# FluidInference/FluidAudio

Measured on NVIDIA H100. Metric: audio-hours/s, higher is better.
Workload: dtype f32

## Files before the change

fluidaudio_b200/csrc/mel_core.cuh:

```cuda
#pragma once

#include "fa_common.cuh"
#include <math.h>
#include <stdint.h>

namespace fa {
namespace mel {

constexpr int kNfft = 512;
constexpr int kHalf = 256;
constexpr int kBins = 257;
constexpr int kFftPad = 304;
constexpr int kTileFrames = 16;
constexpr int kWarpsPerCta = 8;
constexpr int kPairStride = 524;
FA_HD int pow_pos(int bin) { return bin ^ ((bin >> 4) & 3); }

struct alignas(8) cpx {
    float x, y;
};

struct alignas(8) f32x2 {
    float a, b;
};

#if defined(__CUDA_ARCH__)
__device__ __forceinline__ float2 as_f2(f32x2 v) { return make_float2(v.a, v.b); }
__device__ __forceinline__ f32x2 as_v(float2 v) {
    f32x2 r;
    r.a = v.x;
    r.b = v.y;
    return r;
}
#endif

FA_HD double vadd(double x, double y) { return x + y; }
FA_HD double vsub(double x, double y) { return x - y; }
FA_HD double vneg(double x) { return -x; }
FA_HD double vmul_s(double x, double s) { return x * s; }
FA_HD double vfma_s(double a, double s, double c) { return a * s + c; }
FA_HD double vfnma_s(double a, double s, double c) { return c - a * s; }

FA_HD f32x2 vneg(f32x2 x) {
    f32x2 r;
    r.a = -x.a;
    r.b = -x.b;
    return r;
}
#if defined(__CUDA_ARCH__)
__device__ __forceinline__ f32x2 vadd(f32x2 x, f32x2 y) { return as_v(fadd2_rn(as_f2(x), as_f2(y))); }
__device__ __forceinline__ f32x2 vsub(f32x2 x, f32x2 y) { return as_v(fadd2_rn(as_f2(x), as_f2(vneg(y)))); }
__device__ __forceinline__ f32x2 vmul_s(f32x2 x, float s) { return as_v(fmul2_rn(as_f2(x), make_float2(s, s))); }
__device__ __forceinline__ f32x2 vfma_s(f32x2 a, float s, f32x2 c) {
    return as_v(ffma2_rn(as_f2(a), make_float2(s, s), as_f2(c)));
}
__device__ __forceinline__ f32x2 vfnma_s(f32x2 a, float s, f32x2 c) {
    return as_v(ffma2_rn(as_f2(vneg(a)), make_float2(s, s), as_f2(c)));
}
#else
inline f32x2 vadd(f32x2 x, f32x2 y) { return f32x2{x.a + y.a, x.b + y.b}; }
inline f32x2 vsub(f32x2 x, f32x2 y) { return f32x2{x.a - y.a, x.b - y.b}; }
inline f32x2 vmul_s(f32x2 x, float s) { return f32x2{x.a * s, x.b * s}; }
inline f32x2 vfma_s(f32x2 a, float s, f32x2 c) { return f32x2{fmaf(a.a, s, c.a), fmaf(a.b, s, c.b)}; }
inline f32x2 vfnma_s(f32x2 a, float s, f32x2 c) { return f32x2{fmaf(-a.a, s, c.a), fmaf(-a.b, s, c.b)}; }
#endif

template <typename V>
struct vtraits;
template <>
struct vtraits<double> {
    typedef double scalar;
    static constexpr int kFrames = 1;
};
template <>
struct vtraits<f32x2> {
    typedef float scalar;
    static constexpr int kFrames = 2;
};

template <typename V>
struct alignas(16) cpxv {
    V x, y;
};
typedef cpxv<double> cpxd;
struct cpxs {
    float x, y;
};

struct LaneCommon {
    float win[16];
    uint32_t in_win;
    int a1, a2, k0;
    int k0s, kc0s;
};
template <typename V>
struct LaneTables;
template <>
struct LaneTables<double> : LaneCommon {
    cpxd w256;
    cpxd w32;
    cpxd wk0;
};
template <>
struct LaneTables<f32x2> : LaneCommon {
    cpxs tw1[8];
    cpxs tw2[8];
    cpxs wk[4];
};

FA_HD void lane_butterflies(int l, int &c1, int &c2) {
    if (l >= 8) {
        c1 = l;
        c2 = 8 * (8 - (l >> 3)) + (7 - (l & 7));
    } else if (l >= 4) {
        c1 = 32 + (l - 4);
        c2 = 39 - (l - 4);
    } else if (l >= 1) {
        c1 = l;
        c2 = 8 - l;
    } else {
        c1 = 0;
        c2 = 4;
    }
}

FA_HD cpxd unit_root(int k, int n) {
    const double a = -6.283185307179586476925286766559 * (double)k / (double)n;
    cpxd r;
    r.x = cos(a);
    r.y = sin(a);
    return r;
}
FA_HD cpxs unit_root_f(int k, int n) {
    const cpxd d = unit_root(k, n);
    cpxs r;
    r.x = (float)d.x;
    r.y = (float)d.y;
    return r;
}

FA_HD void load_lane_common(int l, const float *win_tab, const uint8_t *in_tab, LaneCommon &T) {
    T.in_win = 0;
#pragma unroll
    for (int r = 0; r < 8; ++r) {
        const int j = 2 * (l + 32 * r);
        T.win[2 * r] = win_tab[j];
        T.win[2 * r + 1] = win_tab[j + 1];
        if (in_tab[j]) T.in_win |= 1u << (2 * r);
        if (in_tab[j + 1]) T.in_win |= 1u << (2 * r + 1);
    }
    int c1, c2;
    lane_butterflies(l, c1, c2);
    T.a1 = 9 * (c1 >> 3) + (c1 & 7);
    T.a2 = 9 * (c2 >> 3) + (c2 & 7);
    T.k0 = (c1 >> 3) + 8 * (c1 & 7);
    T.k0s = pow_pos(T.k0);
    T.kc0s = pow_pos(kHalf - T.k0);
}
FA_HD void load_lane_tables(int l, const float *win_tab, const uint8_t *in_tab, LaneTables<double> &T) {
    load_lane_common(l, win_tab, in_tab, T);
    T.w256 = unit_root(l, 256);
    T.w32 = unit_root(l & 3, 32);
    T.wk0 = unit_root(T.k0, 512);
}
FA_HD void load_lane_tables(int l, const float *win_tab, const uint8_t *in_tab, LaneTables<f32x2> &T) {
    load_lane_common(l, win_tab, in_tab, T);
#pragma unroll
    for (int q = 0; q < 8; ++q) {
        T.tw1[q] = unit_root_f((l * q) & 255, 256);
        T.tw2[q] = unit_root_f(((l & 3) * q) & 31, 32);
    }
#pragma unroll
    for (int k2 = 0; k2 < 4; ++k2) T.wk[k2] = unit_root_f(T.k0 + 64 * k2, 512);
}

FA_HD cpxd cmul(cpxd a, cpxd b) {
    cpxd r;
    r.x = a.x * b.x - a.y * b.y;
    r.y = a.x * b.y + a.y * b.x;
    return r;
}

template <typename V>
FA_HD void dft4(V &r0, V &i0, V &r1, V &i1, V &r2, V &i2, V &r3, V &i3) {
    const V ar = vadd(r0, r2), ai = vadd(i0, i2);
    const V br = vsub(r0, r2), bi = vsub(i0, i2);
    const V cr = vadd(r1, r3), ci = vadd(i1, i3);
    const V dr = vsub(r1, r3), di = vsub(i1, i3);
    r0 = vadd(ar, cr);
    i0 = vadd(ai, ci);
    r2 = vsub(ar, cr);
    i2 = vsub(ai, ci);
    r1 = vadd(br, di);
    i1 = vsub(bi, dr);
    r3 = vsub(br, di);
    i3 = vadd(bi, dr);
}

template <typename V>
FA_HD void dft8(V (&re)[8], V (&im)[8]) {
    typedef typename vtraits<V>::scalar S;
    const S kS = (S)0.70710678118654752440;
    V er0 = vadd(re[0], re[4]), ei0 = vadd(im[0], im[4]);
    V er1 = vadd(re[1], re[5]), ei1 = vadd(im[1], im[5]);
    V er2 = vadd(re[2], re[6]), ei2 = vadd(im[2], im[6]);
    V er3 = vadd(re[3], re[7]), ei3 = vadd(im[3], im[7]);
    V or0 = vsub(re[0], re[4]), oi0 = vsub(im[0], im[4]);
    const V xr1 = vsub(re[1], re[5]), xi1 = vsub(im[1], im[5]);
    const V xr2 = vsub(re[2], re[6]), xi2 = vsub(im[2], im[6]);
    const V xr3 = vsub(re[3], re[7]), xi3 = vsub(im[3], im[7]);
    V or1 = vmul_s(vadd(xr1, xi1), kS), oi1 = vmul_s(vsub(xi1, xr1), kS);
    V or2 = xi2, oi2 = vneg(xr2);
    V or3 = vmul_s(vsub(xi3, xr3), kS), oi3 = vmul_s(vadd(xr3, xi3), (S)(-kS));
    dft4(er0, ei0, er1, ei1, er2, ei2, er3, ei3);
    dft4(or0, oi0, or1, oi1, or2, oi2, or3, oi3);
    re[0] = er0; im[0] = ei0;
    re[2] = er1; im[2] = ei1;
    re[4] = er2; im[4] = ei2;
    re[6] = er3; im[6] = ei3;
    re[1] = or0; im[1] = oi0;
    re[3] = or1; im[3] = oi1;
    re[5] = or2; im[5] = oi2;
    re[7] = or3; im[7] = oi3;
}

template <typename Emit>
FA_HD void twiddle_emit(double (&re)[8], double (&im)[8], cpxd root, Emit emit) {
    cpxd p[8];
    p[1] = root;
    p[2] = cmul(root, root);
    p[3] = cmul(p[2], root);
    p[4] = cmul(p[2], p[2]);
    p[5] = cmul(p[4], root);
    p[6] = cmul(p[4], p[2]);
    p[7] = cmul(p[4], p[3]);
    cpxd v;
    v.x = re[0];
    v.y = im[0];
    emit(0, v);
#pragma unroll
    for (int q = 1; q < 8; ++q) {
        v.x = re[q] * p[q].x - im[q] * p[q].y;
        v.y = re[q] * p[q].y + im[q] * p[q].x;
        emit(q, v);
    }
}
template <typename Emit>
FA_HD void twiddle_emit(f32x2 (&re)[8], f32x2 (&im)[8], const cpxs (&tw)[8], Emit emit) {
    cpxv<f32x2> v;
    v.x = re[0];
    v.y = im[0];
    emit(0, v);
#pragma unroll
    for (int q = 1; q < 8; ++q) {
        v.x = vfnma_s(im[q], tw[q].y, vmul_s(re[q], tw[q].x));
        v.y = vfma_s(im[q], tw[q].x, vmul_s(re[q], tw[q].y));
        emit(q, v);
    }
}
FA_HD void twiddle_pass1(int l, double (&re)[8], double (&im)[8], const LaneTables<double> &T, cpxd *buf) {
    twiddle_emit(re, im, T.w256, [&](int q, cpxd v) { buf[l + 36 * q] = v; });
}
FA_HD void twiddle_pass1(int l, f32x2 (&re)[8], f32x2 (&im)[8], const LaneTables<f32x2> &T, cpxv<f32x2> *buf) {
    twiddle_emit(re, im, T.tw1, [&](int q, cpxv<f32x2> v) { buf[l + 36 * q] = v; });
}
FA_HD void twiddle_pass2(int base, double (&re)[8], double (&im)[8], const LaneTables<double> &T, cpxd *buf) {
    twiddle_emit(re, im, T.w32, [&](int q2, cpxd v) { buf[base + q2] = v; });
}
FA_HD void twiddle_pass2(int base, f32x2 (&re)[8], f32x2 (&im)[8], const LaneTables<f32x2> &T, cpxv<f32x2> *buf) {
    twiddle_emit(re, im, T.tw2, [&](int q2, cpxv<f32x2> v) { buf[base + q2] = v; });
}

FA_HD void widen(float a, float b, float, float, double &re, double &im) {
    re = (double)a;
    im = (double)b;
}
FA_HD void widen(float a, float b, float a2, float b2, f32x2 &re, f32x2 &im) {
    re.a = a;
    re.b = a2;
    im.a = b;
    im.b = b2;
}

template <bool kMidFull, typename V>
FA_HD void pass1(int l, const float *pf, int hop, const LaneTables<V> &T, cpxv<V> *buf) {
    V re[8], im[8];
#pragma unroll
    for (int r = 0; r < 8; ++r) {
        const int j = 2 * (l + 32 * r);
#if defined(__CUDA_ARCH__)
        const float2 v = *reinterpret_cast<const float2 *>(pf + j);
        float2 u = v;
        if (vtraits<V>::kFrames == 2) u = *reinterpret_cast<const float2 *>(pf + hop + j);
#else
        const cpx v = *reinterpret_cast<const cpx *>(pf + j);
        cpx u = v;
        if (vtraits<V>::kFrames == 2) u = *reinterpret_cast<const cpx *>(pf + hop + j);
#endif
        float a = T.win[2 * r] * v.x, b = T.win[2 * r + 1] * v.y;
        float a2 = T.win[2 * r] * u.x, b2 = T.win[2 * r + 1] * u.y;
        if (!kMidFull || r == 0 || r == 7) {
            const bool ia = (T.in_win >> (2 * r)) & 1u, ib = (T.in_win >> (2 * r + 1)) & 1u;
            a = ia ? a : 0.0f;
            b = ib ? b : 0.0f;
            a2 = ia ? a2 : 0.0f;
            b2 = ib ? b2 : 0.0f;
        }
        widen(a, b, a2, b2, re[r], im[r]);
    }
    dft8(re, im);
    twiddle_pass1(l, re, im, T, buf);
}

template <typename V>
FA_HD void pass2_load(int l, const cpxv<V> *buf, V (&re)[8], V (&im)[8]) {
    const int base = 36 * (l >> 2) + (l & 3);
#pragma unroll
    for (int r = 0; r < 8; ++r) {
        const cpxv<V> v = buf[base + 4 * r];
        re[r] = v.x;
        im[r] = v.y;
    }
}
template <typename V>
FA_HD void pass2_store(int l, const LaneTables<V> &T, V (&re)[8], V (&im)[8], cpxv<V> *buf) {
    dft8(re, im);
    const int base = 74 * (l & 3) + 9 * (l >> 2);
    twiddle_pass2(base, re, im, T, buf);
}

FA_HD void pair_power(double zbx, double zby, double zcx, double zcy, double wx, double wy, float *prow, int ib, int ic) {
    const double sr = zbx + zcx, si = zby - zcy;
    const double dr = zby + zcy, di = zcx - zbx;
    const double tr = wx * dr - wy * di, ti = wx * di + wy * dr;
    const float xr = (float)(sr + tr), xi = (float)(si + ti);
    const float yr = (float)(sr - tr), yi = (float)(si - ti);
#if defined(__CUDA_ARCH__)
    prow[2 * ib] = __fadd_rn(__fmul_rn(xr, xr), __fmul_rn(xi, xi));
    prow[2 * ic] = __fadd_rn(__fmul_rn(yr, yr), __fmul_rn(yi, yi));
#else
    const float a = xr * xr, b = xi * xi, c = yr * yr, d = yi * yi;
    prow[2 * ib] = a + b;
    prow[2 * ic] = c + d;
#endif
}
FA_HD void pair_power(f32x2 zbx, f32x2 zby, f32x2 zcx, f32x2 zcy, float wx, float wy, float *prow, int ib, int ic) {
    const f32x2 sr = vadd(zbx, zcx), si = vsub(zby, zcy);
    const f32x2 dr = vadd(zby, zcy), di = vsub(zcx, zbx);
    const f32x2 tr = vfnma_s(di, wy, vmul_s(dr, wx)), ti = vfma_s(dr, wy, vmul_s(di, wx));
    const f32x2 xr = vadd(sr, tr), xi = vadd(si, ti);
    const f32x2 yr = vsub(sr, tr), yi = vsub(si, ti);
#if defined(__CUDA_ARCH__)
    const float2 pb = ffma2_rn(as_f2(xr), as_f2(xr), fmul2_rn(as_f2(xi), as_f2(xi)));
    const float2 pc = ffma2_rn(as_f2(yr), as_f2(yr), fmul2_rn(as_f2(yi), as_f2(yi)));
    *reinterpret_cast<float2 *>(prow + 2 * ib) = pb;
    *reinterpret_cast<float2 *>(prow + 2 * ic) = pc;
#else
    prow[2 * ib] = fmaf(xr.a, xr.a, xi.a * xi.a);
    prow[2 * ic] = fmaf(yr.a, yr.a, yi.a * yi.a);
    prow[2 * ib + 1] = fmaf(xr.b, xr.b, xi.b * xi.b);
    prow[2 * ic + 1] = fmaf(yr.b, yr.b, yi.b * yi.b);
#endif
}

FA_HD void recombination_roots(const LaneTables<double> &T, double (&wx)[4], double (&wy)[4]) {
    const double hh = 0.70710678118654752440;
    wx[0] = T.wk0.x;
    wy[0] = T.wk0.y;
    wx[1] = hh * (wx[0] + wy[0]);
    wy[1] = hh * (wy[0] - wx[0]);
    wx[2] = wy[0];
    wy[2] = -wx[0];
    wx[3] = wy[1];
    wy[3] = -wx[1];
}
FA_HD void recombination_roots(const LaneTables<f32x2> &T, float (&wx)[4], float (&wy)[4]) {
#pragma unroll
    for (int k = 0; k < 4; ++k) {
        wx[k] = T.wk[k].x;
        wy[k] = T.wk[k].y;
    }
}

template <typename V>
FA_HD void pass3_post(int l, const cpxv<V> *buf, const LaneTables<V> &T, float *prow) {
    typedef typename vtraits<V>::scalar S;
    V ar[4], ai[4], br[4], bi[4];
#pragma unroll
    for (int h = 0; h < 4; ++h) {
        const cpxv<V> u = buf[T.a1 + 74 * h], v = buf[T.a2 + 74 * h];
        ar[h] = u.x;
        ai[h] = u.y;
        br[h] = v.x;
        bi[h] = v.y;
    }
    dft4(ar[0], ai[0], ar[1], ai[1], ar[2], ai[2], ar[3], ai[3]);
    dft4(br[0], bi[0], br[1], bi[1], br[2], bi[2], br[3], bi[3]);
    const bool z = l == 0;
    const S c1 = (S)0.92387953251128675613, s1 = (S)0.38268343236508977173;
    S wx[4], wy[4];
    recombination_roots(T, wx, wy);
    pair_power(ar[0], ai[0], z ? ar[0] : br[3], z ? ai[0] : bi[3], wx[0], wy[0], prow, T.k0s, T.kc0s);
    pair_power(ar[1], ai[1], z ? ar[3] : br[2], z ? ai[3] : bi[2], wx[1], wy[1], prow, T.k0s + 64, T.kc0s - 64);
    pair_power(ar[2], ai[2], z ? ar[2] : br[1], z ? ai[2] : bi[1], wx[2], wy[2], prow, T.k0s + 128, T.kc0s - 128);
    const int b3 = z ? pow_pos(32) : T.k0s + 192, c3 = z ? pow_pos(224) : T.kc0s - 192;
    pair_power(z ? br[0] : ar[3], z ? bi[0] : ai[3], z ? br[3] : br[0], z ? bi[3] : bi[0], z ? c1 : wx[3],
               z ? (S)(-s1) : wy[3], prow, b3, c3);
    if (z) {
        pair_power(br[1], bi[1], br[2], bi[2], s1, (S)(-c1), prow, pow_pos(96), pow_pos(160));
    }
}

FA_HD float mel_dot(const float *prow, const float *w, int lo, int hi) {
    float acc = 0.0f;
    const float *p = prow + lo;
    const int n = hi - lo;
    for (int b = 0; b < n; ++b) {
        const float t = w[b] * p[b];
        acc = acc + t;
    }
    return acc;
}
#if defined(__CUDACC__)
__device__ __forceinline__ float2 mel_dot_pairs(const float4 *p4, const float4 *w4, int nq) {
    float2 acc = make_float2(0.0f, 0.0f);
#pragma unroll 1
    for (int b = 0; b < nq; ++b) {
        const float4 x01 = p4[2 * b], x23 = p4[2 * b + 1], c = w4[b];
        acc = ffma2_rn(make_float2(x01.x, x01.y), make_float2(c.x, c.x), acc);
        acc = ffma2_rn(make_float2(x01.z, x01.w), make_float2(c.y, c.y), acc);
        acc = ffma2_rn(make_float2(x23.x, x23.y), make_float2(c.z, c.z), acc);
        acc = ffma2_rn(make_float2(x23.z, x23.w), make_float2(c.w, c.w), acc);
    }
    return acc;
}
__device__ __forceinline__ float mel_dot_quads(const float4 *p4, const float4 *w4, int nq) {
    float acc = 0.0f;
#pragma unroll 1
    for (int b = 0; b < nq; ++b) {
        const float4 x = p4[b], c = w4[b];
        acc = fmaf(c.x, x.x, acc);
        acc = fmaf(c.y, x.y, acc);
        acc = fmaf(c.z, x.z, acc);
        acc = fmaf(c.w, x.w, acc);
    }
    return acc;
}
#endif

FA_HD float log_value(float v, float floor_, int clamped, int normal_floor = 0) {
    const float x = clamped ? (floor_ >= v ? floor_ : v) : v + floor_;
#if defined(__CUDA_ARCH__)
    float l;
    if (normal_floor) asm("lg2.approx.ftz.f32 %0, %1;" : "=f"(l) : "f"(x));
    else l = __log2f(x);
    return l * 0.693147180559945309417f;
#else
    (void)normal_floor;
    return logf(x);
#endif
}

FA_HD float preemph_first(float x0, float last, float a) {
#if defined(__CUDA_ARCH__)
    return __fsub_rn(x0, __fmul_rn(a, last));
#else
    const float t = a * last;
    return x0 - t;
#endif
}
FA_HD float preemph_rest(float x, float xprev, float a) { return fmaf(xprev, -a, x); }

FA_HD long long reflect_index(long long i, long long n) {
    if (i < 0) return -i < n - 1 ? -i : n - 1;
    if (i >= n) return 2 * n - 2 - i > 0 ? 2 * n - 2 - i : 0;
    return i;
}

}
}
```

fluidaudio_b200/csrc/mel_kernels.cu:

```cuda
#include "mel_core.cuh"
#include "mel_plan.h"

#include <cuda_runtime.h>
#include <algorithm>
#include <cmath>
#include <vector>

namespace fa {
namespace mel {

__device__ __forceinline__ uint32_t smem_u32(const void *p) { return (uint32_t)__cvta_generic_to_shared(p); }

__device__ __forceinline__ void mbar_init(uint64_t *bar, uint32_t count) {
    asm volatile("mbarrier.init.shared::cta.b64 [%0], %1;" ::"r"(smem_u32(bar)), "r"(count));
}
__device__ __forceinline__ void mbar_expect_tx(uint64_t *bar, uint32_t bytes) {
    asm volatile("mbarrier.arrive.expect_tx.shared::cta.b64 _, [%0], %1;" ::"r"(smem_u32(bar)), "r"(bytes) : "memory");
}
__device__ __forceinline__ void mbar_arrive(uint64_t *bar) {
    asm volatile("mbarrier.arrive.shared::cta.b64 _, [%0];" ::"r"(smem_u32(bar)) : "memory");
}
__device__ __forceinline__ bool mbar_try_wait(uint64_t *bar, uint32_t parity) {
    uint32_t ok;
    asm volatile(
        "{\n\t"
        ".reg .pred p;\n\t"
        "mbarrier.try_wait.parity.shared::cta.b64 p, [%1], %2;\n\t"
        "selp.u32 %0, 1, 0, p;\n\t"
        "}"
        : "=r"(ok)
        : "r"(smem_u32(bar)), "r"(parity)
        : "memory");
    return ok != 0;
}
__device__ __forceinline__ void mbar_wait(uint64_t *bar, uint32_t parity) {
    while (!mbar_try_wait(bar, parity)) {
    }
}
__device__ __forceinline__ void bulk_g2s(void *dst, const void *src, uint32_t bytes, uint64_t *bar) {
    asm volatile("cp.async.bulk.shared::cluster.global.mbarrier::complete_tx::bytes [%0], [%1], %2, [%3];" ::"r"(
                     smem_u32(dst)),
                 "l"(src), "r"(bytes), "r"(smem_u32(bar))
                 : "memory");
}
__device__ __forceinline__ void fence_proxy_async() { asm volatile("fence.proxy.async.shared::cta;" ::: "memory"); }

struct TileGeom {
    int unit;
    long long f0;
    int nf;
    long long a0;
    long long base;
    long long gs, ge;
};

__device__ __forceinline__ const MelUnit &unit_at(const MelLaunch &P, int idx) { return P.inline_unit ? P.unit0 : P.units[idx]; }

__device__ __forceinline__ TileGeom tile_geom(const MelLaunch &P, int tile) {
    int lo = 0, hi = P.inline_unit ? 0 : P.num_units - 1;
    while (lo < hi) {
        const int mid = (lo + hi + 1) >> 1;
        if (P.units[mid].tile_begin <= tile) lo = mid; else hi = mid - 1;
    }
    const MelUnit &u = P.inline_unit ? P.unit0 : P.units[lo];
    TileGeom g;
    g.unit = lo;
    g.f0 = u.frame_begin + (long long)kTileFrames * (tile - u.tile_begin);
    const long long rem = u.frame_begin + u.frame_count - g.f0;
    g.nf = rem < kTileFrames ? (int)rem : kTileFrames;
    g.a0 = g.f0 * P.hop - P.pad;
    const long long need0 = g.a0 - 1;
    g.base = (need0 >= 0) ? (need0 & ~3LL) : -(((-need0) + 3) & ~3LL);
    long long ge = (g.a0 + P.pt_len + 3) & ~3LL;
    const long long n4 = u.n & ~3LL;
    if (ge > n4) ge = n4;
    g.gs = g.base < 0 ? 0 : g.base;
    g.ge = ge;
    if (!P.use_tma) g.ge = g.gs;
    return g;
}

struct TileInfo {
    TileGeom g;
    long long audio_off, n, out_off, out_stride;
    float last;
    int pad_;
};
__device__ __forceinline__ void make_tile_info(const MelLaunch &P, int tile, TileInfo &ti) {
    ti.g = tile_geom(P, tile);
    const MelUnit &u = unit_at(P, ti.g.unit);
    ti.audio_off = u.audio_off;
    ti.n = u.n;
    ti.out_off = u.out_off;
    ti.out_stride = u.out_stride;
    ti.last = u.last;
}

template <int kWarps, typename V, int kLayout>
__global__ void __launch_bounds__(kWarps * 32, 2) mel512_kernel(const MelLaunch P) {
    constexpr int kF = vtraits<V>::kFrames;
    extern __shared__ __align__(128) unsigned char smem[];
    float *raw0 = reinterpret_cast<float *>(smem);
    float *raw1 = raw0 + P.raw_cap;
    float *ptile = raw1 + P.raw_cap;
    cpxv<V> *fftbuf = reinterpret_cast<cpxv<V> *>(ptile + P.pt_cap);
    float *power = reinterpret_cast<float *>(fftbuf + kWarps * kFftPad);
    float *otile = power + (kTileFrames / 2) * kPairStride;
    const int ot_stride = P.ot_stride;
    float *fbw = otile + kTileFrames * ot_stride;
    int4 *fbmeta = reinterpret_cast<int4 *>(fbw + P.fb_cap);
    uint64_t *bars = reinterpret_cast<uint64_t *>(fbmeta + P.n_slots);
    TileInfo *tinfo = reinterpret_cast<TileInfo *>(bars + 2);

    const int tid = threadIdx.x, lane = tid & 31, warp = tid >> 5;

    if (tid == 0) {
        mbar_init(&bars[0], 1);
        mbar_init(&bars[1], 1);
        asm volatile("fence.mbarrier_init.release.cluster;" ::: "memory");
    }
    for (int i = tid; i < P.fb_nnz; i += kWarps * 32) fbw[i] = P.fb_w[i];
    for (int i = tid; i < P.n_slots; i += kWarps * 32) fbmeta[i] = P.fb_slots[i];
    for (int i = tid; i < (kTileFrames / 2) * kPairStride; i += kWarps * 32) power[i] = 0.0f;
    const LaneTables<V> T = reinterpret_cast<const LaneTables<V> *>(P.lane_tab)[lane];
    __syncthreads();

    cpxv<V> *buf = fftbuf + warp * kFftPad;

    auto issue = [&](int tile, int buf, TileInfo &slot) {
        make_tile_info(P, tile, slot);
        const TileGeom &g = slot.g;
        float *dst = buf ? raw1 : raw0;
        if (g.ge > g.gs) {
            const uint32_t bytes = (uint32_t)((g.ge - g.gs) * 4);
            mbar_expect_tx(&bars[buf], bytes);
            bulk_g2s(dst + (g.gs - g.base), P.audio + slot.audio_off + g.gs, bytes, &bars[buf]);
        } else {
            mbar_arrive(&bars[buf]);
        }
    };

    auto preemphasize = [&](const TileInfo &u, const float *raw) {
        const TileGeom &g = u.g;
        const float a = P.preemph;
        const bool interior = g.a0 >= 1 && g.a0 - 1 >= g.gs && g.a0 + P.pt_len <= g.ge && g.a0 + P.pt_len <= u.n;
        if (interior) {
            const float *src = raw + (g.a0 - g.base);
            if (((g.a0 - g.base) & 3) == 0 && (P.pt_len & 3) == 0) {
                const float4 *s4 = reinterpret_cast<const float4 *>(src);
                float4 *d4 = reinterpret_cast<float4 *>(ptile);
                for (int q = tid; q < (P.pt_len >> 2); q += kWarps * 32) {
                    const float4 x = s4[q];
                    float4 y = x;
                    const float prev = src[4 * q - 1];
                    if (a != 0.0f) {
                        y.x = preemph_rest(x.x, prev, a);
                        y.y = preemph_rest(x.y, x.x, a);
                        y.z = preemph_rest(x.z, x.y, a);
                        y.w = preemph_rest(x.w, x.z, a);
                    }
                    d4[q] = y;
                }
            } else if (a == 0.0f) {
                for (int t = tid; t < P.pt_len; t += kWarps * 32) ptile[t] = src[t];
            } else {
                for (int t = tid; t < P.pt_len; t += kWarps * 32) ptile[t] = preemph_rest(src[t], src[t - 1], a);
            }
        } else {
            const float *gaudio = P.audio + u.audio_off;
            auto sample = [&](long long i) -> float {
                if (i >= g.gs && i < g.ge) return raw[i - g.base];
                if (i < 0) return u.last;
                return __ldg(gaudio + i);
            };
            for (int t = tid; t < P.pt_len; t += kWarps * 32) {
                const long long i = g.a0 + t;
                float v = 0.0f;
                if (i >= 0 && i < u.n) {
                    const float x = sample(i);
                    if (a == 0.0f) v = x;
                    else if (i == 0) v = preemph_first(x, u.last, a);
                    else v = preemph_rest(x, sample(i - 1), a);
                }
                ptile[t] = v;
            }
        }
    };
    auto copy_out = [&](float *dst, int total) {
        if (P.out_vec4) {
            float4 *d4 = reinterpret_cast<float4 *>(dst);
            for (int q = tid; q < (total >> 2); q += kWarps * 32) {
                const int e = 4 * q;
                const int row = (int)__umulhi((unsigned)e, P.inv_n_mels);
                d4[q] = *reinterpret_cast<const float4 *>(otile + e + 4 * row);
            }
        } else {
            const int row_pad = ot_stride - P.n_mels;
            for (int idx = tid; idx < total; idx += kWarps * 32) {
                const int fi = P.n_mels == 1 ? idx : (int)__umulhi((unsigned)idx, P.inv_n_mels);
                dst[idx] = otile[idx + fi * row_pad];
            }
        }
    };

    const int first = blockIdx.x, stride = gridDim.x;
    if (first >= P.total_tiles) return;
    if (tid == 0) {
        issue(first, 0, tinfo[0]);
        if (first + stride < P.total_tiles) issue(first + stride, 1, tinfo[1]);
    }
    __syncthreads();
    mbar_wait(&bars[0], 0);
    preemphasize(tinfo[0], raw0);
    __syncthreads();
    float *pending_dst = nullptr;
    int pending_total = 0;
    int it = 0, slot = 0;
    for (int tile = first; tile < P.total_tiles; tile += stride, ++it, slot = slot == 2 ? 0 : slot + 1) {
        const TileInfo &u = tinfo[slot];
        const int nf = u.g.nf;

        if (pending_dst) copy_out(pending_dst, pending_total);
        for (int fi = warp * kF; fi < nf; fi += kWarps * kF) {
            const float *pf = ptile + fi * P.hop;
            V re[8], im[8];
            if (P.mid_full) pass1<true>(lane, pf, P.hop, T, buf); else pass1<false>(lane, pf, P.hop, T, buf);
            __syncwarp();
            pass2_load(lane, buf, re, im);
            __syncwarp();
            pass2_store(lane, T, re, im, buf);
            __syncwarp();
            pass3_post(lane, buf, T, power + (fi >> 1) * kPairStride + (fi & 1));
            __syncwarp();
        }
        __syncthreads();

        const int next = tile + stride;
        const int slot1 = slot == 2 ? 0 : slot + 1, slot2 = slot1 == 2 ? 0 : slot1 + 1;
        if (tid == 0 && next + stride < P.total_tiles) {
            fence_proxy_async();
            issue(next + stride, it & 1, tinfo[slot2]);
        }
        {
            constexpr int kPairs = kTileFrames / 2, kGroup = 32 / kPairs;
            const int pl = lane % kPairs, mg = lane / kPairs;
            const float *prow = power + pl * kPairStride;
            float *orow = otile + (2 * pl) * ot_stride;
            float *gout = kLayout == 1 ? P.out + u.out_off + u.g.f0 + 2 * pl : nullptr;
            for (int slot = warp * kGroup + mg; slot < P.n_slots; slot += kWarps * kGroup) {
                const int4 md = fbmeta[slot];
                const float2 a2 = mel_dot_pairs(reinterpret_cast<const float4 *>(prow + 2 * md.x),
                                                reinterpret_cast<const float4 *>(fbw + md.z), md.y);
                const float v0 = log_value(a2.x, P.log_floor, P.log_clamped, P.log_normal),
                            v1 = log_value(a2.y, P.log_floor, P.log_clamped, P.log_normal);
                const int m = md.w;
                if (m < 0) continue;
                if (kLayout == 0) {
                    orow[m] = v0;
                    orow[ot_stride + m] = v1;
                } else {
                    float *g = gout + (long long)m * u.out_stride;
                    if (2 * pl < nf) g[0] = v0;
                    if (2 * pl + 1 < nf) g[1] = v1;
                }
            }
        }
        if (kLayout == 0) {
            pending_dst = P.out + u.out_off + u.g.f0 * P.n_mels;
            pending_total = nf * P.n_mels;
        }
        if (next < P.total_tiles) {
            const int nb = (it + 1) & 1;
            mbar_wait(&bars[nb], (uint32_t)((it + 1) >> 1) & 1u);
            preemphasize(tinfo[slot1], nb ? raw1 : raw0);
        }
        __syncthreads();
    }
    if (pending_dst) copy_out(pending_dst, pending_total);
}


struct GenericParams {
    int n_fft, log2n, bins, prow;
    const cpxd *tw;
    int warps;
    float spectrum_power;
    float log_mean, log_std;
};

template <bool kReflect, int kSpectrum, bool kAffine>
__global__ void __launch_bounds__(256) mel_generic_kernel(const MelLaunch P, const GenericParams G) {
    extern __shared__ __align__(16) unsigned char smem[];
    cpxd *tw = reinterpret_cast<cpxd *>(smem);
    cpxd *fft = tw + G.n_fft / 2;
    float *power = reinterpret_cast<float *>(fft + (size_t)G.warps * G.n_fft);
    float *win = power + (size_t)G.warps * G.prow;
    const int tid = threadIdx.x, lane = tid & 31, warp = tid >> 5, nthreads = G.warps * 32;
    for (int i = tid; i < G.n_fft / 2; i += nthreads) tw[i] = G.tw[i];
    for (int i = tid; i < G.n_fft; i += nthreads) win[i] = P.in_tab[i] ? P.win_tab[i] : 0.0f;
    for (int i = tid; i < G.warps * G.prow; i += nthreads) power[i] = 0.0f;
    __syncthreads();
    cpxd *buf = fft + (size_t)warp * G.n_fft;
    float *prow = power + (size_t)warp * G.prow;
    const float a = P.preemph;
    for (int tile = blockIdx.x; tile < P.total_tiles; tile += gridDim.x) {
        const TileGeom g = tile_geom(P, tile);
        const MelUnit u = unit_at(P, g.unit);
        const float *x = P.audio + u.audio_off;
        for (int fi = warp; fi < g.nf; fi += G.warps) {
            const long long f = g.f0 + fi;
            const long long base = f * P.hop - P.pad;
            for (int j = lane; j < G.n_fft; j += 32) {
                const long long i = base + j;
                float v = 0.0f;
                if (kReflect) {
                    if (u.n > 0 && P.in_tab[j]) v = __fmul_rn(__ldg(x + reflect_index(i, u.n)), win[j]);
                } else if (i >= 0 && i < u.n && P.in_tab[j]) {
                    const float xi = __ldg(x + i);
                    if (a == 0.0f) v = xi;
                    else if (i == 0) v = preemph_first(xi, u.last, a);
                    else v = preemph_rest(xi, __ldg(x + i - 1), a);
                    v = __fmul_rn(v, win[j]);
                }
                cpxd z;
                z.x = (double)v;
                z.y = 0.0;
                buf[__brev((unsigned)j) >> (32 - G.log2n)] = z;
            }
            __syncwarp();
            for (int s = 0; s < G.log2n; ++s) {
                const int half = 1 << s, step = G.n_fft >> (s + 1);
                for (int t = lane; t < G.n_fft / 2; t += 32) {
                    const int j = t & (half - 1);
                    const int ia = ((t >> s) << (s + 1)) + j, ib = ia + half;
                    const cpxd w = tw[j * step], zb = buf[ib], za = buf[ia];
                    const double tr = zb.x * w.x - zb.y * w.y, ti = zb.x * w.y + zb.y * w.x;
                    cpxd o;
                    o.x = za.x - tr;
                    o.y = za.y - ti;
                    buf[ib] = o;
                    o.x = za.x + tr;
                    o.y = za.y + ti;
                    buf[ia] = o;
                }
                __syncwarp();
            }
            for (int b = lane; b < G.bins; b += 32) {
                const float xr = (float)buf[b].x, xi = (float)buf[b].y;
                const float pw = __fadd_rn(__fmul_rn(xr, xr), __fmul_rn(xi, xi));
                if (kSpectrum == kSpecPower) prow[b] = 4.0f * pw;
                else if (kSpectrum == kSpecMagnitude) prow[b] = __fsqrt_rn(pw);
                else prow[b] = powf(__fsqrt_rn(pw), G.spectrum_power);
            }
            __syncwarp();
            for (int m = lane; m < P.n_mels; m += 32) {
                const int lo = P.fb_lo[m], nq = (P.fb_hi[m] - lo) >> 2;
                float v = log_value(mel_dot_quads(reinterpret_cast<const float4 *>(prow + lo),
                                                  reinterpret_cast<const float4 *>(P.fb_w + P.fb_off[m]), nq),
                                    P.log_floor, P.log_clamped);
                if (kAffine) v = __fdiv_rn(__fsub_rn(v, G.log_mean), G.log_std);
                if (P.layout == 0) P.out[u.out_off + f * P.n_mels + m] = v;
                else P.out[u.out_off + (long long)m * u.out_stride + f] = v;
            }
            __syncwarp();
        }
    }
}

static constexpr int kCtasPerSm = 2;

typedef void (*Mel512Kernel)(const MelLaunch);
template <typename V> static Mel512Kernel mel512_variant(int layout) {
    return layout == FA_MEL_TIME_MAJOR ? mel512_kernel<kWarpsPerCta, V, FA_MEL_TIME_MAJOR>
                                       : mel512_kernel<kWarpsPerCta, V, FA_MEL_MEL_MAJOR>;
}
static Mel512Kernel mel512_variant(int precision, int layout) {
    return precision == FA_MEL_PRECISION_F64 ? mel512_variant<double>(layout) : mel512_variant<f32x2>(layout);
}

typedef void (*GenericKernel)(const MelLaunch, const GenericParams);
template <bool R, int S> static GenericKernel generic_variant(bool affine) {
    return affine ? mel_generic_kernel<R, S, true> : mel_generic_kernel<R, S, false>;
}
template <bool R> static GenericKernel generic_variant(int spectrum, bool affine) {
    return spectrum == kSpecPower ? generic_variant<R, kSpecPower>(affine)
                                  : (spectrum == kSpecMagnitude ? generic_variant<R, kSpecMagnitude>(affine)
                                                                : generic_variant<R, kSpecGeneral>(affine));
}
static GenericKernel generic_variant(bool reflect, int spectrum, bool affine) {
    return reflect ? generic_variant<true>(spectrum, affine) : generic_variant<false>(spectrum, affine);
}

static int placement_of(int mode) { return mode == FA_MEL_LEGACY_COMPUTE ? 1 : 0; }
static int window_offset(const MelConfig &c, int placement) { return placement == 1 ? 0 : (c.n_fft - c.win_length) / 2; }

static_assert(sizeof(MelSlot) == sizeof(int4) && offsetof(MelSlot, mel) == offsetof(int4, w), "MelSlot is an int4");

template <typename T, typename U> static int upload_table(DeviceBuffer<T> &b, const std::vector<U> &v) {
    const int st = b.grow(std::max<size_t>(1, v.size()) * sizeof(U));
    if (st != FA_OK) return st;
    if (!v.empty()) FA_CUDA_TRY(cudaMemcpy(b.data(), v.data(), v.size() * sizeof(U), cudaMemcpyHostToDevice));
    return FA_OK;
}

int MelPlan::init(const MelConfig &c) {
    cfg = c;
    if (cfg.pad_to < 1) cfg.pad_to = 1;
    if (cfg.n_mels <= 0 || cfg.hop_length <= 0 || cfg.win_length <= 0 || cfg.n_fft <= 0 || cfg.sample_rate <= 0) {
        fa::set_error("mel config: all sizes must be positive");
        return FA_INVALID_ARGUMENT;
    }
    const bool pow2 = cfg.n_fft >= 32 && cfg.n_fft <= 4096 && (cfg.n_fft & (cfg.n_fft - 1)) == 0;
    if (!pow2 || cfg.win_length > cfg.n_fft || cfg.n_mels > 512 || cfg.hop_length > 65536) {
        fa::set_error("mel config unsupported by the sm_90a kernels: need nFFT a power of two in 32..4096, win <= nFFT, "
                      "nMels <= 512 (got nFFT=%d hop=%d win=%d nMels=%d)",
                      cfg.n_fft, cfg.hop_length, cfg.win_length, cfg.n_mels);
        return FA_UNSUPPORTED;
    }
    if (const char *why = check_ex_config(cfg)) {
        fa::set_error("mel ex config: %s", why);
        return FA_INVALID_ARGUMENT;
    }
    const int spectrum = spectrum_kind(cfg.spectrum_power);
    generic = cfg.n_fft != kNfft || (cfg.hop_length & 1) || cfg.hop_length > 1024 || cfg.reflect() ||
              spectrum != kSpecPower || cfg.affine();
    const int n_fft = cfg.n_fft, bins = n_fft / 2 + 1;
    build_tables(cfg, window, filterbank);
    const MelBands bands = pack_bands(filterbank, cfg.n_mels, bins);
    fb_nnz = bands.nnz;
    n_slots = (int)bands.slots.size();

    int dev = 0;
    FA_CUDA_TRY(cudaGetDevice(&dev));
    cudaDeviceProp prop;
    int st = sm90_device_props(dev, prop);
    if (st != FA_OK) return st;
    num_sms = prop.multiProcessorCount;

    if (!generic) {
        pt_len = (kTileFrames - 1) * cfg.hop_length + kNfft;
        pt_cap = (pt_len + 31) & ~31;
        raw_cap = (pt_len + 1 + 3 + 3 + 31) & ~31;
        fb_cap = (fb_nnz + 3) & ~3;
        smem_bytes = sizeof(float) * ((size_t)2 * raw_cap + pt_cap + 0 +
                                      (size_t)(kTileFrames / 2) * kPairStride + (size_t)kTileFrames * (cfg.n_mels + 4) + fb_cap) +
                     sizeof(cpxd) * (size_t)kWarpsPerCta * kFftPad + sizeof(int) * 4 * (size_t)n_slots + 8 +
                     2 * sizeof(uint64_t) + 3 * sizeof(TileInfo) + 16;
        if (smem_bytes > (size_t)prop.sharedMemPerBlockOptin) {
            generic = true;
            pt_len = pt_cap = raw_cap = fb_cap = 0;
        }
    }

    std::vector<float> win_tab;
    std::vector<uint8_t> in_tab;
    for (int pl = 0; pl < 2; ++pl) {
        place_window(window, n_fft, window_offset(cfg, pl), win_tab, in_tab);
        st = upload_table(d_win_tab_mode[pl], win_tab);
        if (st == FA_OK) st = upload_table(d_in_tab_mode[pl], in_tab);
        if (st != FA_OK) return st;
        if (!generic) {
            std::vector<LaneTables<double>> t64(32);
            std::vector<LaneTables<f32x2>> t32(32);
            for (int l = 0; l < 32; ++l) {
                load_lane_tables(l, win_tab.data(), in_tab.data(), t64[l]);
                load_lane_tables(l, win_tab.data(), in_tab.data(), t32[l]);
            }
            st = upload_table(d_lane_tab[pl][FA_MEL_PRECISION_F64], t64);
            if (st == FA_OK) st = upload_table(d_lane_tab[pl][FA_MEL_PRECISION_F32], t32);
            if (st != FA_OK) return st;
        }
    }
    st = upload_table(d_fb_w, pack_weights(filterbank, bands, bins, !generic, spectrum == kSpecPower ? 0.25f : 1.0f));
    if (st == FA_OK) st = upload_table(d_fb_slots, bands.slots);
    if (st == FA_OK) st = upload_table(d_fb_lo, bands.lo);
    if (st == FA_OK) st = upload_table(d_fb_hi, bands.hi);
    if (st == FA_OK) st = upload_table(d_fb_off, bands.off);
    for (auto &s : streams)
        if (st == FA_OK) st = s.create();
    if (st != FA_OK) return st;
    if (generic) {
        std::vector<cpxd> tw(n_fft / 2);
        for (int k = 0; k < n_fft / 2; ++k) tw[k] = unit_root(k, n_fft);
        st = upload_table(d_generic_tw, tw);
        if (st != FA_OK) return st;
        generic_prow = ((bins + 3) & ~3) + 4;
        int log2n = 0;
        while ((1 << log2n) < n_fft) ++log2n;
        generic_log2n = log2n;
        const size_t fixed = (size_t)(n_fft / 2) * sizeof(cpxd) + (size_t)n_fft * sizeof(float);
        const size_t per_warp = (size_t)n_fft * sizeof(cpxd) + (size_t)generic_prow * sizeof(float);
        generic_warps = (int)std::min<size_t>(8, ((size_t)prop.sharedMemPerBlockOptin - fixed - 1024) / per_warp);
        if (generic_warps < 1) {
            fa::set_error("mel config: nFFT %d does not fit shared memory", n_fft);
            return FA_UNSUPPORTED;
        }
        smem_bytes = fixed + per_warp * generic_warps;
        for (const bool r : {false, cfg.reflect()})
            FA_CUDA_TRY(cudaFuncSetAttribute(generic_variant(r, spectrum, cfg.affine()),
                                             cudaFuncAttributeMaxDynamicSharedMemorySize, (int)smem_bytes));
        return FA_OK;
    }
    for (const int precision : {FA_MEL_PRECISION_F64, FA_MEL_PRECISION_F32})
        for (const int layout : {FA_MEL_TIME_MAJOR, FA_MEL_MEL_MAJOR})
            FA_CUDA_TRY(cudaFuncSetAttribute(mel512_variant(precision, layout), cudaFuncAttributeMaxDynamicSharedMemorySize,
                                             (int)smem_bytes));
    return FA_OK;
}

long long MelPlan::frame_count(long long n, int mode, long long expected) const {
    long long computed;
    if (mode == FA_MEL_PAD_CENTER) computed = 1 + (n + 2 * (long long)(cfg.n_fft / 2) - cfg.win_length) / cfg.hop_length;
    else if (mode == FA_MEL_PAD_PREPADDED) computed = std::max<long long>(0, (n - cfg.n_fft) / cfg.hop_length + 1);
    else computed = 1 + (n - cfg.win_length) / cfg.hop_length;
    return expected >= 0 ? expected : computed;
}

int MelPlan::ensure_staging(size_t audio_floats, size_t out_floats) {
    const int st = d_audio.grow(audio_floats * sizeof(float));
    return st != FA_OK ? st : d_out.grow(out_floats * sizeof(float));
}

int MelPlan::ensure_events(size_t count) {
    while (events.size() < count) {
        Event e;
        const int st = e.create(cudaEventDisableTiming);
        if (st != FA_OK) return st;
        events.push_back(std::move(e));
    }
    return FA_OK;
}

static int tiles_of(long long frames) { return (int)((frames + kTileFrames - 1) / kTileFrames); }

int number_tiles(MelUnit *u, int count) {
    int tiles = 0;
    for (int i = 0; i < count; ++i) {
        u[i].tile_begin = tiles;
        tiles += tiles_of(u[i].frame_count);
    }
    return tiles;
}

int MelPlan::launch(const MelUnit *d_u, const MelUnit *h_u, int count, bool inline_unit, const float *d_audio_base,
                    float *d_out_base, int mode, int layout, cudaStream_t stream) {
    const int total_tiles = count > 0 ? h_u[count - 1].tile_begin + tiles_of(h_u[count - 1].frame_count) : 0;
    if (total_tiles <= 0) return FA_OK;
    MelLaunch P{};
    P.audio = d_audio_base;
    P.out = d_out_base;
    P.units = d_u;
    P.num_units = count;
    P.inline_unit = (inline_unit && count == 1) ? 1 : 0;
    if (P.inline_unit) P.unit0 = h_u[0];
    P.total_tiles = total_tiles;
    P.hop = cfg.hop_length;
    P.pad = mode == FA_MEL_PAD_CENTER ? cfg.n_fft / 2 : 0;
    P.preemph = mode == FA_MEL_LEGACY_COMPUTE ? 0.0f : cfg.preemph;
    P.n_mels = cfg.n_mels;
    P.log_floor = cfg.log_floor;
    P.log_clamped = cfg.log_floor_mode;
    P.ot_stride = (cfg.n_mels & 3) == 0 ? cfg.n_mels + 4 : cfg.n_mels + 1;
    P.out_vec4 = (cfg.n_mels & 3) == 0 && (reinterpret_cast<uintptr_t>(d_out_base) & 15) == 0;
    for (int i = 0; i < count && P.out_vec4; ++i) P.out_vec4 = (h_u[i].out_off & 3) == 0;
    P.log_normal = cfg.log_floor >= 1e-37f ? 1 : 0;
    P.layout = layout;
    const int pl = placement_of(mode);
    P.lane_tab = d_lane_tab[pl][precision == FA_MEL_PRECISION_F32 ? 1 : 0].data();
    P.win_tab = d_win_tab_mode[pl].data();
    P.in_tab = d_in_tab_mode[pl].data();
    P.fb_w = d_fb_w.data();
    P.fb_slots = d_fb_slots.data();
    P.n_slots = n_slots;
    P.fb_lo = d_fb_lo.data();
    P.fb_hi = d_fb_hi.data();
    P.fb_off = d_fb_off.data();
    P.fb_nnz = fb_nnz;
    P.fb_cap = fb_cap;
    P.pt_len = pt_len;
    P.pt_cap = pt_cap;
    P.raw_cap = raw_cap;
    P.use_tma = (reinterpret_cast<uintptr_t>(d_audio_base) & 15) == 0;
    for (int i = 0; i < count && P.use_tma; ++i) P.use_tma = (h_u[i].audio_off & 3) == 0;
    {
        const int off_w = window_offset(cfg, pl);
        P.mid_full = (off_w <= 64 && off_w + cfg.win_length >= 448) ? 1 : 0;
    }
    P.inv_n_mels = (unsigned)((0x100000000ull + (unsigned)cfg.n_mels - 1) / (unsigned)cfg.n_mels);
    if (generic) {
        GenericParams G{cfg.n_fft, generic_log2n, cfg.n_fft / 2 + 1, generic_prow,
                        static_cast<const cpxd *>(d_generic_tw.data()), generic_warps, cfg.spectrum_power, cfg.log_mean,
                        cfg.log_std};
        const int ggrid = std::min(total_tiles, num_sms * std::max(1, 16 / generic_warps));
        const GenericKernel kernel = generic_variant(mode == FA_MEL_PAD_CENTER && cfg.reflect(),
                                                     spectrum_kind(cfg.spectrum_power), cfg.affine());
        FA_CUDA_TRY(fa::launch(kernel, ggrid, generic_warps * 32, smem_bytes, stream, P, G));
        return FA_OK;
    }
    const int grid = std::min(total_tiles, num_sms * kCtasPerSm);
    const dim3 blk(kWarpsPerCta * 32);
    FA_CUDA_TRY(fa::launch(mel512_variant(precision, layout), grid, blk, smem_bytes, stream, P));
    return FA_OK;
}

static bool shape_of(const MelPlan &p, long long n, int mode, long long expected, long long &T, long long &Tp) {
    T = p.frame_count(n, mode, mode == FA_MEL_PAD_CENTER || mode == FA_MEL_PAD_PREPADDED ? expected : -1);
    if (T <= 0 || n <= 0) return false;
    Tp = mode == FA_MEL_LEGACY_COMPUTE ? T : ceil_to(T, p.cfg.pad_to);
    return true;
}

int clip_shape(const MelPlan &p, long long n, int mode, long long expected, long long out_len, long long &T,
               long long &Tp, long long *mel_length, long long *num_frames) {
    if (!shape_of(p, n, mode, expected, T, Tp)) {
        T = 0;
        Tp = mode == FA_MEL_LEGACY_COMPUTE ? 0 : 1;
    }
    if (mel_length) *mel_length = T;
    if (num_frames) *num_frames = Tp;
    if (out_len < Tp * p.cfg.n_mels) {
        fa::set_error("mel output needs %lld floats, buffer has %lld", Tp * p.cfg.n_mels, out_len);
        return FA_OUTPUT_TOO_SMALL;
    }
    return FA_OK;
}

int MelPlan::compute_device(const float *d_in, long long n, float last, int mode, long long expected, int layout,
                            float *d_out_buf, long long out_len, long long *mel_length, long long *num_frames,
                            cudaStream_t stream) {
    long long T, Tp;
    int st = clip_shape(*this, n, mode, expected, out_len, T, Tp, mel_length, num_frames);
    if (st != FA_OK) return st;
    if (T == 0) {
        if (Tp) FA_CUDA_TRY(cudaMemsetAsync(d_out_buf, 0, cfg.n_mels * sizeof(float), stream));
        return FA_OK;
    }
    st = units.reserve(unit_bytes(1));
    if (st != FA_OK) return st;
    if (Tp > T) FA_CUDA_TRY(cudaMemsetAsync(d_out_buf, 0, Tp * cfg.n_mels * sizeof(float), stream));
    units.host.data()[0] = MelUnit{0, n, 0, Tp, 0, T, last, 0};
    st = units.upload(sizeof(MelUnit), stream);
    if (st != FA_OK) return st;
    return launch(units.device.data(), units.host.data(), 1, false, d_in, d_out_buf, mode, layout, stream);
}

int MelPlan::launch_clip(const float *d_in, long long n, long long T, int layout, float *d_out_buf, cudaStream_t stream) {
    if (T <= 0) return FA_OK;
    int st = units.reserve(unit_bytes(1));
    if (st != FA_OK) return st;
    units.host.data()[0] = MelUnit{0, n, 0, T, 0, T, 0.0f, 0};
    st = units.upload(sizeof(MelUnit), stream);
    if (st != FA_OK) return st;
    return launch(units.device.data(), units.host.data(), 1, false, d_in, d_out_buf, FA_MEL_PAD_CENTER, layout, stream);
}

int MelPlan::compute_batch_device(const float *d_in, const long long *offsets, int count, const float *last, int mode,
                                  int layout, float *d_out_buf, const long long *out_offsets, long long *mel_lengths,
                                  long long *num_frames, cudaStream_t stream) {
    int st = units.reserve(unit_bytes(count));
    if (st != FA_OK) return st;
    MelUnit *h_units = units.host.data();
    int used = 0;
    for (int i = 0; i < count; ++i) {
        const long long n = offsets[i + 1] - offsets[i];
        long long T, Tp;
        clip_shape(*this, n, mode, -1, kUnchecked, T, Tp, mel_lengths ? mel_lengths + i : nullptr,
                   num_frames ? num_frames + i : nullptr);
        if (T == 0) {
            if (Tp) FA_CUDA_TRY(cudaMemsetAsync(d_out_buf + out_offsets[i], 0, cfg.n_mels * sizeof(float), stream));
            continue;
        }
        if (Tp > T) FA_CUDA_TRY(cudaMemsetAsync(d_out_buf + out_offsets[i], 0, Tp * cfg.n_mels * sizeof(float), stream));
        h_units[used++] = MelUnit{offsets[i], n, out_offsets[i], Tp, 0, T, last ? last[i] : 0.0f, 0};
    }
    if (!used) return FA_OK;
    number_tiles(h_units, used);
    st = units.upload(used * sizeof(MelUnit), stream);
    if (st != FA_OK) return st;
    return launch(units.device.data(), h_units, used, false, d_in, d_out_buf, mode, layout, stream);
}

}
}
```

Baseline: 3100.

## Specialize log flags, skip dead mel slots early, pass single unit inline

The mel dot-product stage is turned into a lambda that is instantiated for each combination of the clamped and normal log flags, so log_value sees compile-time constants. The dead-slot check now runs before the dot product instead of after it. Preemphasis gets a separate copy-only loop for a zero coefficient, and the filterbank dot loop uses pointer increments. Single-clip launches pass the unit inline (the `true` flag) rather than reserving and uploading a device buffer, which removes an H2D copy per call. The cost is four template instantiations and more code size.

Measured after the change: 3187, median of 6. 1.03x the previous value.

```diff
diff --git a/fluidaudio_b200/csrc/mel_core.cuh b/fluidaudio_b200/csrc/mel_core.cuh
--- a/fluidaudio_b200/csrc/mel_core.cuh
+++ b/fluidaudio_b200/csrc/mel_core.cuh
@@ -425,8 +425,8 @@
 __device__ __forceinline__ float2 mel_dot_pairs(const float4 *p4, const float4 *w4, int nq) {
     float2 acc = make_float2(0.0f, 0.0f);
 #pragma unroll 1
-    for (int b = 0; b < nq; ++b) {
-        const float4 x01 = p4[2 * b], x23 = p4[2 * b + 1], c = w4[b];
+    for (const float4 *const end = w4 + nq; w4 != end; ++w4, p4 += 2) {
+        const float4 x01 = p4[0], x23 = p4[1], c = *w4;
         acc = ffma2_rn(make_float2(x01.x, x01.y), make_float2(c.x, c.x), acc);
         acc = ffma2_rn(make_float2(x01.z, x01.w), make_float2(c.y, c.y), acc);
         acc = ffma2_rn(make_float2(x23.x, x23.y), make_float2(c.z, c.z), acc);
diff --git a/fluidaudio_b200/csrc/mel_kernels.cu b/fluidaudio_b200/csrc/mel_kernels.cu
--- a/fluidaudio_b200/csrc/mel_kernels.cu
+++ b/fluidaudio_b200/csrc/mel_kernels.cu
@@ -96,6 +96,8 @@
     ti.last = u.last;
 }
 
+template <int v> using Flag = std::integral_constant<int, v>;
+
 template <int kWarps, typename V, int kLayout>
 __global__ void __launch_bounds__(kWarps * 32, 2) mel512_kernel(const MelLaunch P) {
     constexpr int kF = vtraits<V>::kFrames;
@@ -149,17 +151,19 @@
             if (((g.a0 - g.base) & 3) == 0 && (P.pt_len & 3) == 0) {
                 const float4 *s4 = reinterpret_cast<const float4 *>(src);
                 float4 *d4 = reinterpret_cast<float4 *>(ptile);
-                for (int q = tid; q < (P.pt_len >> 2); q += kWarps * 32) {
-                    const float4 x = s4[q];
-                    float4 y = x;
-                    const float prev = src[4 * q - 1];
-                    if (a != 0.0f) {
+                if (a == 0.0f) {
+                    for (int q = tid; q < (P.pt_len >> 2); q += kWarps * 32) d4[q] = s4[q];
+                } else {
+                    for (int q = tid; q < (P.pt_len >> 2); q += kWarps * 32) {
+                        const float4 x = s4[q];
+                        const float prev = src[4 * q - 1];
+                        float4 y;
                         y.x = preemph_rest(x.x, prev, a);
                         y.y = preemph_rest(x.y, x.x, a);
                         y.z = preemph_rest(x.z, x.y, a);
                         y.w = preemph_rest(x.w, x.z, a);
+                        d4[q] = y;
                     }
-                    d4[q] = y;
                 }
             } else if (a == 0.0f) {
                 for (int t = tid; t < P.pt_len; t += kWarps * 32) ptile[t] = src[t];
@@ -203,6 +207,31 @@
         }
     };
 
+    auto mel_stage = [&](const TileInfo &u, int nf, auto clamped, auto normal_floor) {
+        constexpr int kPairs = kTileFrames / 2, kGroup = 32 / kPairs;
+        const int pl = lane % kPairs, mg = lane / kPairs;
+        const float *prow = power + pl * kPairStride;
+        float *orow = otile + (2 * pl) * ot_stride;
+        float *gout = kLayout == 1 ? P.out + u.out_off + u.g.f0 + 2 * pl : nullptr;
+        for (int slot = warp * kGroup + mg; slot < P.n_slots; slot += kWarps * kGroup) {
+            const int4 md = fbmeta[slot];
+            const int m = md.w;
+            if (m < 0) continue;
+            const float2 a2 = mel_dot_pairs(reinterpret_cast<const float4 *>(prow + 2 * md.x),
+                                            reinterpret_cast<const float4 *>(fbw + md.z), md.y);
+            const float v0 = log_value(a2.x, P.log_floor, clamped.value, normal_floor.value),
+                        v1 = log_value(a2.y, P.log_floor, clamped.value, normal_floor.value);
+            if (kLayout == 0) {
+                orow[m] = v0;
+                orow[ot_stride + m] = v1;
+            } else {
+                float *g = gout + (long long)m * u.out_stride;
+                if (2 * pl < nf) g[0] = v0;
+                if (2 * pl + 1 < nf) g[1] = v1;
+            }
+        }
+    };
+
     const int first = blockIdx.x, stride = gridDim.x;
     if (first >= P.total_tiles) return;
     if (tid == 0) {
@@ -241,29 +270,10 @@
             fence_proxy_async();
             issue(next + stride, it & 1, tinfo[slot2]);
         }
-        {
-            constexpr int kPairs = kTileFrames / 2, kGroup = 32 / kPairs;
-            const int pl = lane % kPairs, mg = lane / kPairs;
-            const float *prow = power + pl * kPairStride;
-            float *orow = otile + (2 * pl) * ot_stride;
-            float *gout = kLayout == 1 ? P.out + u.out_off + u.g.f0 + 2 * pl : nullptr;
-            for (int slot = warp * kGroup + mg; slot < P.n_slots; slot += kWarps * kGroup) {
-                const int4 md = fbmeta[slot];
-                const float2 a2 = mel_dot_pairs(reinterpret_cast<const float4 *>(prow + 2 * md.x),
-                                                reinterpret_cast<const float4 *>(fbw + md.z), md.y);
-                const float v0 = log_value(a2.x, P.log_floor, P.log_clamped, P.log_normal),
-                            v1 = log_value(a2.y, P.log_floor, P.log_clamped, P.log_normal);
-                const int m = md.w;
-                if (m < 0) continue;
-                if (kLayout == 0) {
-                    orow[m] = v0;
-                    orow[ot_stride + m] = v1;
-                } else {
-                    float *g = gout + (long long)m * u.out_stride;
-                    if (2 * pl < nf) g[0] = v0;
-                    if (2 * pl + 1 < nf) g[1] = v1;
-                }
-            }
+        if (P.log_clamped) {
+            if (P.log_normal) mel_stage(u, nf, Flag<1>{}, Flag<1>{}); else mel_stage(u, nf, Flag<1>{}, Flag<0>{});
+        } else {
+            if (P.log_normal) mel_stage(u, nf, Flag<0>{}, Flag<1>{}); else mel_stage(u, nf, Flag<0>{}, Flag<0>{});
         }
         if (kLayout == 0) {
             pending_dst = P.out + u.out_off + u.g.f0 * P.n_mels;
@@ -635,23 +645,15 @@
         if (Tp) FA_CUDA_TRY(cudaMemsetAsync(d_out_buf, 0, cfg.n_mels * sizeof(float), stream));
         return FA_OK;
     }
-    st = units.reserve(unit_bytes(1));
-    if (st != FA_OK) return st;
     if (Tp > T) FA_CUDA_TRY(cudaMemsetAsync(d_out_buf, 0, Tp * cfg.n_mels * sizeof(float), stream));
-    units.host.data()[0] = MelUnit{0, n, 0, Tp, 0, T, last, 0};
-    st = units.upload(sizeof(MelUnit), stream);
-    if (st != FA_OK) return st;
-    return launch(units.device.data(), units.host.data(), 1, false, d_in, d_out_buf, mode, layout, stream);
+    const MelUnit u{0, n, 0, Tp, 0, T, last, 0};
+    return launch(nullptr, &u, 1, true, d_in, d_out_buf, mode, layout, stream);
 }
 
 int MelPlan::launch_clip(const float *d_in, long long n, long long T, int layout, float *d_out_buf, cudaStream_t stream) {
     if (T <= 0) return FA_OK;
-    int st = units.reserve(unit_bytes(1));
-    if (st != FA_OK) return st;
-    units.host.data()[0] = MelUnit{0, n, 0, T, 0, T, 0.0f, 0};
-    st = units.upload(sizeof(MelUnit), stream);
-    if (st != FA_OK) return st;
-    return launch(units.device.data(), units.host.data(), 1, false, d_in, d_out_buf, FA_MEL_PAD_CENTER, layout, stream);
+    const MelUnit u{0, n, 0, T, 0, T, 0.0f, 0};
+    return launch(nullptr, &u, 1, true, d_in, d_out_buf, FA_MEL_PAD_CENTER, layout, stream);
 }
 
 int MelPlan::compute_batch_device(const float *d_in, const long long *offsets, int count, const float *last, int mode,
```
